# Maboroshi0327/MHAda-Style-Transfer

Measured on AMD Instinct MI355X. Metric: stylized frames/sec (whole job) at 512x512 batch 8 fp32 [configs[1]], higher is better.
Workload: dtype f32; 1 GPU; stylize 512x512 content+style, batch 8; resolution=512, batch_per_gpu=8, global_batch=8, compute_dtype=f32, parallelism=replicas x1

## Files before the change

### include/mhada_hip.h

```cpp
#ifndef MHADA_HIP_H
#define MHADA_HIP_H

#ifdef __cplusplus
extern "C" {
#endif

typedef void* mhada_stream_t;

enum { MHADA_OK = 0, MHADA_ERR_ARG = 1, MHADA_ERR_LAUNCH = 2 };
enum { MHADA_F32 = 0, MHADA_BF16 = 1 };
enum { MHADA_ACT_SOFTMAX = 0, MHADA_ACT_COSINE = 1 };
enum { MHADA_PAD_REFLECT = 0, MHADA_PAD_ZERO = 1 };
enum {
  MHADA_A_ROWS = 0,
  MHADA_A_PATCH8 = 1,
  MHADA_A_CONV3X3 = 2,
  MHADA_A_CONV3X3_UP2 = 3,
  MHADA_A_CONV3X3_ZERO = 4,
  MHADA_A_SPLIT3 = 5
};
enum { MHADA_BF16X3 = 2 };

int mhada_abi_version(void);
const char* mhada_last_error(void);
// ... 126 lines not shown
int mhada_colsum(const float* x, float* out, long long rows, int C, float* work, long long work_floats,
                 mhada_stream_t stream);

int mhada_layernorm_fwd(const float* x, float* y, float* stats, const float* gamma, const float* beta,
                        int rows, int cols, float eps, mhada_stream_t stream);
int mhada_layernorm_fwd_split3(const float* x, float* y, void* planes, float* stats, const float* gamma,
                               const float* beta, int rows, int cols, float eps, mhada_stream_t stream);

int mhada_layernorm_bwd(const float* x, const float* dy, const float* stats, const float* gamma, float* dx,
                        float* dgamma, float* dbeta, float* work, long long work_floats, int rows, int cols,
                        mhada_stream_t stream);

int mhada_instnorm_bwd(const float* dy, const float* y, const float* rstd, float* dx, double* work,
                       int B, int N, int C, int splits, mhada_stream_t stream);

int mhada_attn_train_bwd_prep(const float* dout, const float* x, const float* mo, float* dx, float* dmo,
                              float* dd, long long rows, mhada_stream_t stream);

int mhada_pos_embed_bwd(const float* g, float* gpos, int C, int bh, int bw, int oh, int ow,
                        mhada_stream_t stream);
long long mhada_feat_stats_work(int B, long long P, int C);
int mhada_feat_stats(const float* x, const float* t, float* mu, float* sd, float* mse, double* work,
                     long long work_doubles, int B, long long P, int C, mhada_stream_t stream);
int mhada_feat_loss_bwd(const float* x, const float* t, const float* mu, const float* alpha, const float* beta,
                        const float* kp, float ks, float* g, int B, long long P, int C, int relu, mhada_stream_t stream);
int mhada_relu_bwd(const float* dy, const float* y, float* dx, long long n, mhada_stream_t stream);
int mhada_reflect_fold(const float* dxp, float* dx, int B, int H, int W, int C, const float* relu_mask,
                       mhada_stream_t stream);
int mhada_maxpool2(const float* x, float* y, int B, int H, int W, int C, mhada_stream_t stream);
int mhada_maxpool2_bwd(const float* x, const float* dy, float* dx, int B, int H, int W, int C, int relu_mask,
                       mhada_stream_t stream);
int mhada_upsample2x_bwd(const float* dy, const float* relu_x, float* dx, int B, int H, int W, int C,
                         mhada_stream_t stream);
int mhada_vgg_input(const float* img, float* out, int B, int H, int W, int Cp, mhada_stream_t stream);
int mhada_vgg_input_bwd(const float* dout, float* dimg, int B, int H, int W, int Cp, mhada_stream_t stream);

int mhada_loss_attn(const float* q, const float* k, const float* v, const float* x, const float* x_mu,
                    const float* x_rs, float* out, int B, int Nq, int Ns, int Dqk, int Dv, int activation,
                    mhada_stream_t stream);
int mhada_rows_normalize(const float* x, const float* mu, const float* rs, float* out, int unit,
                         int B, int N, int C, mhada_stream_t stream);

int mhada_frame_ingest(const void* frames, int B, int H, int W, long long row_bytes, int bgr, float* out,
                       int Ho, int Wo, mhada_stream_t stream);

int mhada_wino_weights(const float* w, float* u, int Cout, int Cin, mhada_stream_t stream);
int mhada_conv3x3_wgrad_wino_splits(int B, int H, int W, int Cin, int Cout);
int mhada_conv3x3_wgrad_wino(const float* x, const float* g, float* dw, float* db, float* work, long long work_floats,
                             int B, int H, int W, int Cin, int Cout, long long ldg, int pad_mode,
                             mhada_stream_t stream);
int mhada_conv3x3_wino(const float* x, const float* u, const float* bias, float* y, int B, int H, int W,
                       int Cin, int Cout, long long ldc, int pad_mode, int pad, int relu,
                       const float* relu_mask, mhada_stream_t stream);

int mhada_vgg_stem_dgrad(const float* dy, const float* y, const float* wd, float* dimg, int B, int H, int W,
                         mhada_stream_t stream);
int mhada_out3_dgrad(const float* dy, const float* y, const float* wd, const float* relu_x, float* dx, int B, int H,
                     int W, mhada_stream_t stream);
long long mhada_out3_wgrad_work(int B, int H, int W);
int mhada_out3_wgrad(const float* x, const float* dy, const float* y, float* dw, float* db, float* work,
                     long long work_floats, int B, int H, int W, mhada_stream_t stream);

#ifdef __cplusplus
}
#endif
#endif
```

### mhada-style-transfer_amd/csrc/abi.hip

```cpp
#include "common.h"

#include <mutex>
#include <stdlib.h>
#include <string.h>

namespace mhada {

static thread_local std::string g_last_error;

void set_error(const std::string& msg) { g_last_error = msg; }

int fail(const std::string& msg) {
  set_error(msg);
  return MHADA_ERR_ARG;
}

int check_launch(const char* what) {
  const hipError_t e = hipGetLastError();
  if (e != hipSuccess) {
    set_error(std::string(what) + ": " + hipGetErrorString(e));
    return MHADA_ERR_LAUNCH;
  }
  return MHADA_OK;
}

namespace {
struct Knob {
  const char* name;
  int Tuning::*field;
};
const Knob kKnobs[] = {
    {"attn_fixed_shift", &Tuning::attn_fixed_shift}, {"attn_waves", &Tuning::attn_waves},
    {"attn_tk", &Tuning::attn_tk},                   {"attn_prio", &Tuning::attn_prio},
    {"vit_attn_vec", &Tuning::vit_attn_vec},         {"out3_mfma", &Tuning::out3_mfma},
    {"out3_tile", &Tuning::out3_tile},               {"gemm_pp", &Tuning::gemm_pp},
    {"gemm_persist", &Tuning::gemm_persist},         {"gemm_pp128", &Tuning::gemm_pp128},
    {"gemm_ldsepi", &Tuning::gemm_ldsepi},           {"gemm_n64", &Tuning::gemm_n64},
    {"conv_c64", &Tuning::conv_c64},                 {"conv_dir", &Tuning::conv_dir},                 {"gemm_rinit", &Tuning::gemm_rinit},
    {"tn_skinny_lds", &Tuning::tn_skinny_lds},       {"train_dkv_dma", &Tuning::train_dkv_dma},
    {"wino4", &Tuning::wino4},                       {"upsample_quad", &Tuning::upsample_quad},
    {"xknob", &Tuning::xknob},
};

Tuning g_tuning;
std::once_flag g_tuning_once;

void read_env_once() {
  std::call_once(g_tuning_once, [] {
    for (const Knob& k : kKnobs) {
      std::string env = "MHADA_";
      for (const char* c = k.name; *c; ++c) env += (char)(*c >= 'a' && *c <= 'z' ? *c - 32 : *c);
      if (const char* v = getenv(env.c_str())) g_tuning.*k.field = atoi(v);
    }
  });
}

bool valid(const char* name, int v) {
  if (!strcmp(name, "attn_waves")) return v == 0 || v == 4 || v == 8;
  if (!strcmp(name, "attn_tk")) return v == 64 || v == 128;
  if (!strcmp(name, "gemm_n64")) return v == 128 || v == 256;
  if (!strcmp(name, "xknob")) return v >= 0 && v < 16;
  return v == 0 || v == 1;
}
}

const Tuning& tuning() {
  read_env_once();
  return g_tuning;
}

}

extern "C" int mhada_abi_version(void) { return 16; }

extern "C" const char* mhada_last_error(void) { return mhada::g_last_error.c_str(); }

extern "C" int mhada_set_tuning(const char* name, int value) {
  using namespace mhada;
  read_env_once();
  if (!name) return fail("mhada_set_tuning: null name");
  for (const Knob& k : kKnobs) {
    if (!strcmp(k.name, name)) {
      if (!valid(name, value)) return fail(std::string("mhada_set_tuning: bad value for ") + name);
      g_tuning.*k.field = value;
      return MHADA_OK;
    }
  }
  return fail(std::string("mhada_set_tuning: unknown knob ") + name);
}

extern "C" int mhada_get_tuning(const char* name, int* value) {
  using namespace mhada;
  read_env_once();
  if (!name || !value) return fail("mhada_get_tuning: null argument");
  for (const Knob& k : kKnobs) {
    if (!strcmp(k.name, name)) {
      *value = g_tuning.*k.field;
      return MHADA_OK;
    }
  }
  return fail(std::string("mhada_get_tuning: unknown knob ") + name);
}
```

### mhada-style-transfer_amd/csrc/common.h

```cpp
#pragma once
#include <hip/hip_runtime.h>
#include <stdint.h>
#include <string>

#include "../../include/mhada_hip.h"

typedef __bf16 bf16;
typedef __bf16 bf16x8 __attribute__((ext_vector_type(8)));
typedef __bf16 bf16x4 __attribute__((ext_vector_type(4)));
typedef float f32x16 __attribute__((ext_vector_type(16)));
typedef float f32x4 __attribute__((ext_vector_type(4)));
typedef float f32x2 __attribute__((ext_vector_type(2)));

#define MHADA_DEV __device__ __forceinline__

namespace mhada {

void set_error(const std::string& msg);
int fail(const std::string& msg);
int check_launch(const char* what);

struct Tuning {
  int attn_fixed_shift = 1;
  int attn_waves = 0;
  int attn_tk = 128;
  int attn_prio = 1;
  int vit_attn_vec = 1;
  int out3_mfma = 1;
  int out3_tile = 1;
  int gemm_pp = 1;
  int gemm_persist = 1;
  int gemm_pp128 = 1;
  int gemm_ldsepi = 1;
  int gemm_n64 = 128;
  int conv_c64 = 1;
  int conv_dir = 1;
  int gemm_rinit = 1;
  int tn_skinny_lds = 1;
  int wino4 = 1;
  int train_dkv_dma = 1;
  int upsample_quad = 1;
  int xknob = 0;
};
const Tuning& tuning();

int conv3x3_c64(const void* x, const void* w, const float* bias, void* y, int B, int H, int W, bool up, int relu,
                hipStream_t s);
int conv3x3_dir(const void* x, const void* w, const float* bias, void* y, int B, int H, int W, int cin, int cout,
                int relu, hipStream_t s);

template <typename T> MHADA_DEV float to_f32(T x);
template <> MHADA_DEV float to_f32<float>(float x) { return x; }
template <> MHADA_DEV float to_f32<bf16>(bf16 x) { return (float)x; }

template <typename T> MHADA_DEV T from_f32(float x);
template <> MHADA_DEV float from_f32<float>(float x) { return x; }
template <> MHADA_DEV bf16 from_f32<bf16>(float x) { return (bf16)x; }

template <typename T> struct Vec16;
template <> struct Vec16<float> { typedef f32x4 type; static constexpr int N = 4; };
template <> struct Vec16<bf16> { typedef bf16x8 type; static constexpr int N = 8; };

MHADA_DEV float bilerp(float ly0, float ly1, float lx0, float lx1, float x00, float x01, float x10, float x11) {
  return fmaf(ly1, fmaf(lx0, x10, lx1 * x11), ly0 * fmaf(lx0, x00, lx1 * x01));
}

MHADA_DEV float wave_sum(float v) {
#pragma unroll
  for (int o = 32; o > 0; o >>= 1) v += __shfl_xor(v, o, 64);
  return v;
}
MHADA_DEV float wave_max(float v) {
#pragma unroll
  for (int o = 32; o > 0; o >>= 1) v = fmaxf(v, __shfl_xor(v, o, 64));
  return v;
}

MHADA_DEV int xcd_remap(int bid, int nblk) {
  const int q = nblk / 8, r = nblk % 8;
  const int xcd = bid % 8, k = bid / 8;
  return (xcd < r ? xcd * (q + 1) : r * (q + 1) + (xcd - r) * q) + k;
}

}
```

### mhada-style-transfer_amd/csrc/wino.hip

```cpp
#include "common.h"

#include <algorithm>
#include <utility>

#ifndef WINO_DBG
#define WINO_DBG 0
#endif
#ifndef WINO4_DBG
#define WINO4_DBG 0
#endif

namespace mhada {

namespace {
constexpr int kT = 8;
constexpr int kTT = kT * kT;
constexpr int kCO = 64;
constexpr int kCK = 8;
constexpr int kRP = 2 * kT + 2;
constexpr int kRaw = kRP * kRP;
constexpr int kRDma = (2 * kRaw + 63) / 64;
constexpr int kVS = 16 * kTT * kCK;
constexpr int kUS = 16 * kCO * kCK;
constexpr int kRS = kRDma * 64 * 4;
// ... 353 lines not shown
      if constexpr ((DBG & 4) == 0) {
#pragma unroll
        for (int s = 0; s < 4; ++s)
          acc[xi] = __builtin_amdgcn_mfma_f32_32x32x2f32(oa[xi % 3][s], ob[xi % 3][s], acc[xi], 0, 0, 0);
      }
      if (xi < 11) dma_piece(xi, k + 1, N, k + 2, C);
      if (xi == 2) tload(N);
      if (xi == 4) { tcols(); trows(N, 0); }
      if (xi == 5) trows(N, 2);
      fence();
    }
    publish();
  };
  int k = 0;
  for (; k + 1 < nck; k += 2) {
    chunk(k, std::integral_constant<int, 0>());
    chunk(k + 1, std::integral_constant<int, 1>());
  }
  if (k < nck) chunk(k, std::integral_constant<int, 0>());

  const int co = co0 + 32 * ch + r32;
  const float bias = p.bias ? p.bias[co] : 0.f;
#pragma unroll
  for (int r = 0; r < 16; ++r) {
    const int tile = 32 * th + (r & 3) + 8 * (r >> 2) + 4 * h;
    float m[4][2];
#pragma unroll
    for (int i = 0; i < 4; ++i) {
      const float m0 = acc[4 * i][r], m1 = acc[4 * i + 1][r], m2 = acc[4 * i + 2][r], m3 = acc[4 * i + 3][r];
      m[i][0] = m0 + m1 + m2;
      m[i][1] = m1 - m2 - m3;
    }
    const int oy0 = 2 * (by * kT + (tile >> 3)), ox0 = 2 * (bx * kT + (tile & 7));
#pragma unroll
    for (int q = 0; q < 2; ++q) {
      const float e1 = -m[2][q] - m[3][q];
      float y0 = m[0][q] + m[1][q] + m[2][q] + bias;
      float y1 = m[1][q] + e1 + bias;
      if (p.relu) {
        y0 = fmaxf(y0, 0.f);
        y1 = fmaxf(y1, 0.f);
      }
      const int ox = ox0 + q;
      if (ox < p.Wo) {
        const long long i0 = ((long long)(b * p.Ho + oy0) * p.Wo + ox) * p.ldc + co;
        const long long i1 = i0 + (long long)p.Wo * p.ldc;
        if (p.mask) {
          if (oy0 < p.Ho && !(p.mask[i0] > 0.f)) y0 = 0.f;
          if (oy0 + 1 < p.Ho && !(p.mask[i1] > 0.f)) y1 = 0.f;
        }
        if (oy0 < p.Ho) p.y[i0] = y0;
        if (oy0 + 1 < p.Ho) p.y[i1] = y1;
      }
    }
  }
}

__global__ void wino_weights_kernel(const float* __restrict__ w, float* __restrict__ u, int Cout, int Cin) {
  const long long i = (long long)blockIdx.x * blockDim.x + threadIdx.x;
  if (i >= (long long)Cout * Cin) return;
  const int ci = (int)(i % Cin), co = (int)(i / Cin);
  float g[9];
#pragma unroll
  for (int t = 0; t < 9; ++t) g[t] = w[((long long)co * 9 + t) * Cin + ci];
  float gg[12];
#pragma unroll
  for (int kx = 0; kx < 3; ++kx) {
    const float a = g[kx], bb = g[3 + kx], c = g[6 + kx];
    gg[0 * 3 + kx] = a;
    gg[1 * 3 + kx] = 0.5f * (a + bb + c);
    gg[2 * 3 + kx] = 0.5f * (a - bb + c);
    gg[3 * 3 + kx] = c;
  }
  float* ub = u + ((long long)(ci / kCK) * 16 * Cout + co) * kCK + (ci % kCK);
#pragma unroll
  for (int r = 0; r < 4; ++r) {
    const float a = gg[3 * r], bb = gg[3 * r + 1], c = gg[3 * r + 2];
    const float v[4] = {a, 0.5f * (a + bb + c), 0.5f * (a - bb + c), c};
#pragma unroll
    for (int j = 0; j < 4; ++j) ub[(long long)(4 * r + j) * Cout * kCK] = v[j];
  }
}
constexpr int kWgT = 8;
constexpr int kWgS = 16 * 64 * kWgT;
constexpr int kWgRX = 4 * 18 * 64;
constexpr int kWgRY = 2 * 16 * 64;

struct WgP {
  const float* x;
  const float* g;
  float* slab;
  float* cslab;
  int B, H, W, Cin, Cout, zero;
  long long ldg;
  int crow, nchunk, cps;
};

MHADA_DEV int wg_px(int px, int c) { return px * 64 + (c ^ (8 * ((px >> 1) & 7))); }

template <bool ZERO>
__global__ void __launch_bounds__(512, 1) wino_wgrad_kernel(const WgP p) {
  __shared__ __attribute__((aligned(16))) float lds[4 * kWgS + kWgRX + kWgRY];
  auto sYh = [&](int i) { return lds + i * kWgS; };
  auto sVb = [&](int i) { return lds + (2 + i) * kWgS; };
  float* sRX = lds + 4 * kWgS;
  float* sRY = sRX + kWgRX;
// ... 240 lines not shown
  if (B <= 0 || H < 2 || W < 16 || Cin <= 0 || Cout <= 0 || Cin % 64 || Cout % 64) return 0;
  const long long nchunk = (long long)B * (H / 2) * (W / 16);
  const long long blocks = (long long)(Cout / 64) * (Cin / 64);
  const long long s = std::max<long long>(1, std::min<long long>((512 + blocks - 1) / blocks, nchunk / 16));
  return (int)std::min<long long>(s, 65535);
}

extern "C" int mhada_conv3x3_wgrad_wino(const float* x, const float* g, float* dw, float* db, float* work,
                                        long long work_floats, int B, int H, int W, int Cin, int Cout, long long ldg,
                                        int pad_mode, mhada_stream_t s_) {
  if (!x || !g || !dw || !work || B <= 0 || H < 2 || W < 2 || Cin <= 0 || Cout <= 0)
    return fail("mhada_conv3x3_wgrad_wino: bad args");
  if (Cin % 64 || Cout % 64 || H % 2 || W % 16)
    return fail("mhada_conv3x3_wgrad_wino: needs Cin % 64 == 0, Cout % 64 == 0, H even, W % 16 == 0");
  if (pad_mode != MHADA_PAD_REFLECT && pad_mode != MHADA_PAD_ZERO) return fail("mhada_conv3x3_wgrad_wino: bad pad_mode");
  if (ldg < Cout || ldg % 4) return fail("mhada_conv3x3_wgrad_wino: ldg >= Cout, ldg % 4 == 0");
  if (((uintptr_t)x | (uintptr_t)g | (uintptr_t)work) & 15) return fail("mhada_conv3x3_wgrad_wino: 16-byte aligned x, g, work");
  if ((long long)B * H * W * std::max<long long>(Cin, ldg) > (1LL << 31) - 1)
    return fail("mhada_conv3x3_wgrad_wino: problem too large for 32-bit indexing");
  WgP p;
  p.x = x; p.g = g;
  p.B = B; p.H = H; p.W = W; p.Cin = Cin; p.Cout = Cout; p.ldg = ldg;
  p.zero = pad_mode == MHADA_PAD_ZERO;
  p.crow = W / 16;
  p.nchunk = B * (H / 2) * p.crow;
  int S = mhada_conv3x3_wgrad_wino_splits(B, H, W, Cin, Cout);
  const long long per = 16LL * Cout * Cin + (db ? Cout : 0);
  S = (int)std::min<long long>(S, work_floats / per);
  if (S < 1) return fail("mhada_conv3x3_wgrad_wino: workspace smaller than 16*Cout*Cin (+Cout) floats");
  p.cps = (p.nchunk + S - 1) / S;
  S = (p.nchunk + p.cps - 1) / p.cps;
  p.slab = work;
  p.cslab = db ? work + (long long)S * 16 * Cout * Cin : nullptr;
  const dim3 grid((unsigned)((Cout / 64) * (Cin / 64)), (unsigned)S);
  if (p.zero)
    hipLaunchKernelGGL(wino_wgrad_kernel<true>, grid, dim3(512), 0, (hipStream_t)s_, p);
  else
    hipLaunchKernelGGL(wino_wgrad_kernel<false>, grid, dim3(512), 0, (hipStream_t)s_, p);
  if (int rc = check_launch("mhada_conv3x3_wgrad_wino")) return rc;
  const long long n = (long long)Cout * Cin;
  hipLaunchKernelGGL(wino_wgrad_finish_kernel, dim3((unsigned)((n + 255) / 256)), dim3(256), 0, (hipStream_t)s_,
                     p.slab, p.cslab, dw, db, Cout, Cin, S);
  return check_launch("mhada_conv3x3_wgrad_wino(finish)");
}

extern "C" int mhada_wino_weights(const float* w, float* u, int Cout, int Cin, mhada_stream_t s_) {
  if (!w || !u || Cout <= 0 || Cin <= 0 || Cin % kCK) return fail("mhada_wino_weights: bad args (Cin % 8 == 0)");
  const long long n = (long long)Cout * Cin;
  hipLaunchKernelGGL(wino_weights_kernel, dim3((unsigned)((n + 255) / 256)), dim3(256), 0, (hipStream_t)s_, w, u,
                     Cout, Cin);
  return check_launch("mhada_wino_weights");
}

extern "C" int mhada_conv3x3_wino(const float* x, const float* u, const float* bias, float* y, int B, int H, int W,
                                  int Cin, int Cout, long long ldc, int pad_mode, int pad, int relu,
                                  const float* relu_mask, mhada_stream_t s_) {
  if (!x || !u || !y || B <= 0 || H < 2 || W < 2 || Cin <= 0 || Cout <= 0)
    return fail("mhada_conv3x3_wino: bad args");
  if (Cin % kCK || Cout % kCO) return fail("mhada_conv3x3_wino: needs Cin % 8 == 0 and Cout % 64 == 0");
  if (pad_mode != MHADA_PAD_REFLECT && pad_mode != MHADA_PAD_ZERO) return fail("mhada_conv3x3_wino: bad pad_mode");
  if (pad_mode == MHADA_PAD_ZERO && pad != 1 && pad != 2) return fail("mhada_conv3x3_wino: zero pad must be 1 or 2");
  if (ldc < Cout) return fail("mhada_conv3x3_wino: ldc < Cout");
  if (((uintptr_t)x | (uintptr_t)u) & 15) return fail("mhada_conv3x3_wino: x and u must be 16-byte aligned");
  WinoP p;
  p.x = x; p.u = u; p.bias = bias; p.y = y; p.mask = relu_mask;
  p.B = B; p.H = H; p.W = W; p.Cin = Cin; p.Cout = Cout;
  p.zero = pad_mode == MHADA_PAD_ZERO;
  p.pad = p.zero ? pad : 1;
  p.Ho = p.zero ? H + 2 * (pad - 1) : H;
  p.Wo = p.zero ? W + 2 * (pad - 1) : W;
  p.relu = relu;
  p.ldc = ldc;
  const int TY = (p.Ho + 1) / 2, TX = (p.Wo + 1) / 2;
  p.nby = (TY + kT - 1) / kT;
  p.nbx = (TX + kT - 1) / kT;
  p.nbn = Cout / kCO;
  const long long nblk = (long long)B * p.nby * p.nbx * p.nbn;
  if (nblk > (1LL << 31) - 1 || (long long)B * H * W * Cin > (1LL << 31) - 1)
    return fail("mhada_conv3x3_wino: problem too large for 32-bit indexing");
  p.nblk = (int)nblk;
  if (tuning().wino4 && (long long)B * H * W * Cin * 4 < 0x7ff00000LL) {
    hipLaunchKernelGGL(wino4_kernel<WINO4_DBG>, dim3(p.nblk), dim3(256), 0, (hipStream_t)s_, p);
  } else
    hipLaunchKernelGGL(wino_kernel, dim3(p.nblk), dim3(512), 0, (hipStream_t)s_, p);
  return check_launch("mhada_conv3x3_wino");
}
```

### mhada-style-transfer_amd/mhada_hip/_lib.py

```python
from __future__ import annotations

import ctypes
import os
import threading

LIB_PATH = os.path.join(os.path.dirname(os.path.abspath(__file__)), "libmhada_hip.so")

F32, BF16 = 0, 1
ACT_SOFTMAX, ACT_COSINE = 0, 1
A_ROWS, A_PATCH8, A_CONV3X3, A_CONV3X3_UP2, A_CONV3X3_ZERO, A_SPLIT3 = 0, 1, 2, 3, 4, 5
BF16X3 = 2
PAD_REFLECT, PAD_ZERO = 0, 1

_c_ll = ctypes.c_longlong
_vp = ctypes.c_void_p


class GemmArgs(ctypes.Structure):
    _fields_ = [
        ("M", ctypes.c_int), ("N", ctypes.c_int), ("K", ctypes.c_int),
        ("nb1", ctypes.c_int), ("nb2", ctypes.c_int),
        ("compute", ctypes.c_int), ("a_mode", ctypes.c_int),
        ("a", _vp), ("a_dtype", ctypes.c_int), ("lda", _c_ll), ("sa1", _c_ll), ("sa2", _c_ll),
        ("a_mu", _vp), ("smu1", _c_ll), ("smu2", _c_ll),
# ... 34 lines not shown
    "mhada_fold_block": (_I, [_vp] * 12 + [_F, _I, _I, _I, _vp]),
    "mhada_transpose_v": (_I, [_vp, _vp, _I, _I, _I, _I, _vp]),
    "mhada_cosine_prep": (_I, [_vp, _vp, _I, _I, _I, _I, _I, _vp]),
    "mhada_cosine_moments": (_I, [_vp, _vp, _I, _I, _I, _I, _vp, _vp, _I, _vp]),
    "mhada_cosine_attn": (_I, [_vp, _vp, _vp, _vp, _vp, _vp, _vp, _I, _I, _I, _I, _vp]),
    "mhada_attn": (_I, [_vp] * 8 + [_I, _I, _I, _I, _I, _I, _vp]),
    "mhada_split3_kv": (_I, [_vp, _vp, _vp, _I, _I, _I, _vp]),
    "mhada_kv_proj_split3": (_I, [_vp] * 5 + [_I, _I, _I, _vp]),
    "mhada_split3_rows": (_I, [_vp, _vp, _c_ll, _vp]),
    "mhada_split3_weight": (_I, [_vp, _vp, _I, _I, _I, _vp]),
    "mhada_attn_split3": (_I, [_vp] * 7 + [_I, _I, _I, _I, _vp]),
    "mhada_attn_train_fwd": (_I, [_vp] * 7 + [_I, _I, _I, _vp]),
    "mhada_attn_train_fwd_vt": (_I, [_vp] * 8 + [_I, _I, _I, _vp]),
    "mhada_attn_train_fwd_split3": (_I, [_vp] * 8 + [_I, _I, _I, _vp]),
    "mhada_transpose64": (_I, [_vp, _vp, _I, _I, _I, _vp]),
    "mhada_gemm_n64_split3": (_I, [_vp, _vp, _vp, _I, _I, _I, _I, _c_ll, _I, _c_ll, _c_ll, _I, _c_ll, _vp]),
    "mhada_transpose64_split3": (_I, [_vp, _vp, _I, _I, _I, _vp]),
    "mhada_attn_train_bwd": (_I, [_vp] * 9 + [_I, _I, _I, _vp]),
    "mhada_attn_train_dkv": (_I, [_vp] * 9 + [_I, _I, _I, _vp]),
    "mhada_conv3x3_out3": (_I, [_vp, _I, _vp, _vp, _vp, _I, _I, _I, _I, _I, _vp]),
    "mhada_upsample2x": (_I, [_vp, _vp, _I, _I, _I, _I, _I, _vp]),
    "mhada_warp": (_I, [_vp, _vp, _vp, _I, _I, _I, _I, _I, _vp]),
    "mhada_warp_bwd": (_I, [_vp, _vp, _vp, _I, _I, _I, _I, _I, _vp]),
    "mhada_flow_warp_mask": (_I, [_vp, _vp, _vp, _I, _I, _F, _I, _vp]),
    "mhada_warp_l1": (_I, [_vp, _vp, _vp, _vp, _vp, _vp, _I, _I, _I, _I, _vp]),
    "mhada_frame_ingest": (_I, [_vp, _I, _I, _I, _c_ll, _I, _vp, _I, _I, _vp]),
    "mhada_gemm_tn_splits": (_I, [_I, _I, _I]),
    "mhada_loss_attn": (_I, [_vp] * 7 + [_I, _I, _I, _I, _I, _I, _vp]),
    "mhada_rows_normalize": (_I, [_vp] * 4 + [_I, _I, _I, _I, _vp]),
    "mhada_gemm_tn": (_I, [ctypes.POINTER(GemmTnArgs), _vp, _c_ll, _vp]),
    "mhada_colsum": (_I, [_vp, _vp, _c_ll, _I, _vp, _c_ll, _vp]),
    "mhada_layernorm_fwd": (_I, [_vp, _vp, _vp, _vp, _vp, _I, _I, _F, _vp]),
    "mhada_layernorm_fwd_split3": (_I, [_vp, _vp, _vp, _vp, _vp, _vp, _I, _I, _F, _vp]),
    "mhada_layernorm_bwd": (_I, [_vp, _vp, _vp, _vp, _vp, _vp, _vp, _vp, _c_ll, _I, _I, _vp]),
    "mhada_pos_embed_bwd": (_I, [_vp, _vp, _I, _I, _I, _I, _I, _vp]),
    "mhada_instnorm_bwd": (_I, [_vp, _vp, _vp, _vp, _vp, _I, _I, _I, _I, _vp]),
    "mhada_attn_train_bwd_prep": (_I, [_vp, _vp, _vp, _vp, _vp, _vp, _c_ll, _vp]),
    "mhada_vit_batch_attn_bwd": (_I, [_vp, _vp, _vp, _I, _I, _I, _I, _vp]),
    "mhada_vit_batch_attn_bwd_split3": (_I, [_vp, _vp, _vp, _vp, _c_ll, _I, _I, _I, _I, _vp]),
    "mhada_relu_bwd": (_I, [_vp, _vp, _vp, _c_ll, _vp]),
    "mhada_feat_stats_work": (_c_ll, [_I, _c_ll, _I]),
    "mhada_feat_stats": (_I, [_vp, _vp, _vp, _vp, _vp, _vp, _c_ll, _I, _c_ll, _I, _vp]),
    "mhada_feat_loss_bwd": (_I, [_vp, _vp, _vp, _vp, _vp, _vp, _F, _vp, _I, _c_ll, _I, _I, _vp]),
    "mhada_reflect_fold": (_I, [_vp, _vp, _I, _I, _I, _I, _vp, _vp]),
    "mhada_maxpool2": (_I, [_vp, _vp, _I, _I, _I, _I, _vp]),
    "mhada_maxpool2_bwd": (_I, [_vp, _vp, _vp, _I, _I, _I, _I, _I, _vp]),
    "mhada_upsample2x_bwd": (_I, [_vp, _vp, _vp, _I, _I, _I, _I, _vp]),
    "mhada_vgg_input": (_I, [_vp, _vp, _I, _I, _I, _I, _vp]),
    "mhada_vgg_input_bwd": (_I, [_vp, _vp, _I, _I, _I, _I, _vp]),
    "mhada_wino_weights": (_I, [_vp, _vp, _I, _I, _vp]),
    "mhada_conv3x3_wgrad_wino_splits": (_I, [_I, _I, _I, _I, _I]),
    "mhada_conv3x3_wgrad_wino": (_I, [_vp, _vp, _vp, _vp, _vp, _c_ll, _I, _I, _I, _I, _I, _c_ll, _I, _vp]),
    "mhada_conv3x3_wino": (_I, [_vp] * 4 + [_I] * 5 + [_c_ll, _I, _I, _I, _vp, _vp]),
    "mhada_vgg_stem_dgrad": (_I, [_vp] * 4 + [_I] * 3 + [_vp]),
    "mhada_out3_dgrad": (_I, [_vp] * 5 + [_I] * 3 + [_vp]),
    "mhada_out3_wgrad_work": (_c_ll, [_I, _I, _I]),
    "mhada_out3_wgrad": (_I, [_vp] * 6 + [_c_ll, _I, _I, _I, _vp]),
}

_lib = None
_lock = threading.Lock()


def load(path: str | None = None) -> ctypes.CDLL:
    global _lib
    if _lib is not None and path is None:
        return _lib
    with _lock:
        if _lib is not None and path is None:
            return _lib
        p = path or LIB_PATH
        if not os.path.exists(p):
            raise RuntimeError(
                f"MHAda HIP library not found at {p}; build it with "
                "`python -c 'import __graft_entry__ as g; g.build()'` (make -C mhada-style-transfer_amd/csrc)")
        lib = ctypes.CDLL(p)
        for name, (res, args) in SIGNATURES.items():
            fn = getattr(lib, name)
            fn.restype = res
            fn.argtypes = args
        if path is None:
            _lib = lib
        return lib


ABI_VERSION = 16


def get_tuning(name: str) -> int:
    v = ctypes.c_int()
    check(load().mhada_get_tuning(name.encode(), ctypes.byref(v)), "mhada_get_tuning")
    return v.value


def set_tuning(name: str, value: int) -> None:
    check(load().mhada_set_tuning(name.encode(), int(value)), "mhada_set_tuning")


class tuning:

    def __init__(self, **knobs: int):
        self.knobs = knobs
        self.saved = {}

    def __enter__(self):
        for k, v in self.knobs.items():
            self.saved[k] = get_tuning(k)
            set_tuning(k, v)
        return self

    def __exit__(self, *exc):
        for k, v in self.saved.items():
            set_tuning(k, v)
        return False


def check(rc: int, what: str) -> None:
    if rc != 0:
        msg = load().mhada_last_error()
        msg = msg.decode() if msg else "unknown error"
        if rc == 1:
            raise ValueError(f"{what}: {msg}")
        raise RuntimeError(f"{what}: {msg}")
```

### mhada-style-transfer_amd/mhada_hip/ops.py

```python
from __future__ import annotations

import contextlib
import ctypes
from typing import Optional

import torch

from . import _lib
from ._lib import A_CONV3X3, A_CONV3X3_UP2, A_CONV3X3_ZERO, A_PATCH8, A_ROWS, A_SPLIT3, BF16, BF16X3, F32, GemmArgs, GemmTnArgs

_DT = {torch.float32: F32, torch.bfloat16: BF16}


def dt_code(dtype: torch.dtype) -> int:
    try:
        return _DT[dtype]
    except KeyError:
        raise ValueError(f"unsupported dtype {dtype}; the HIP path computes in float32 or bfloat16")


def _ptr(t: Optional[torch.Tensor]) -> Optional[int]:
    return None if t is None else t.data_ptr()


# ... 91 lines not shown


def patch_embed(img: torch.Tensor, w: torch.Tensor, bias: torch.Tensor, pos: Optional[torch.Tensor],
                patch: int = 8) -> torch.Tensor:
    if patch != 8:
        raise ValueError("the HIP patch embedding implements patch_size=8 (the reference default)")
    B, Ci, H, W = img.shape
    h, wd = H // 8, W // 8
    N, C = h * wd, w.shape[0]
    out = torch.empty(B, N, C, device=img.device, dtype=torch.float32)
    return gemm(a=img, w=w, c=out, M=N, N=C, K=Ci * 64, compute=w.dtype, a_mode=A_PATCH8,
                sa=(Ci * H * W, 0), nb=(B, 1), img=(Ci, H, W), ldw=w.stride(0), bias=bias,
                r=pos, ldr=C, sr=(0, 0), ldc=C, sc=(N * C, 0))


WINO = True


def wino_eligible(x: torch.Tensor, w: torch.Tensor, upsample: bool) -> bool:
    return (WINO and w.dtype == torch.float32 and x.dtype == torch.float32 and not upsample
            and x.shape[-1] % 8 == 0 and w.shape[0] % 64 == 0 and x.shape[1] >= 2 and x.shape[2] >= 2
            and x.numel() < 2 ** 31 and x.numel() // x.shape[-1] * w.shape[0] < 2 ** 31)


WINO_WGRAD = True


def wgrad_wino_eligible(x: torch.Tensor, g: torch.Tensor, cout: int) -> bool:
    if not (WINO_WGRAD and x.is_cuda and x.dtype == torch.float32 and g.dtype == torch.float32):
        return False
    B, H, W, ci = x.shape
    return (ci % 64 == 0 and cout % 64 == 0 and H % 2 == 0 and W % 16 == 0 and g.shape[:3] == x.shape[:3]
            and g.shape[3] >= cout and g.shape[3] % 4 == 0 and x.is_contiguous() and g.is_contiguous()
            and B * H * W * max(ci, g.shape[3]) < 2 ** 31)


def conv3x3_wgrad_wino(x: torch.Tensor, g: torch.Tensor, cout: int, pad_mode: str = "reflect",
                       bias: bool = True):
    _need_gpu(x, g)
    B, H, W, ci = x.shape
    lib = _lib.load()
    S = lib.mhada_conv3x3_wgrad_wino_splits(B, H, W, ci, cout)
    if S <= 0:
        raise ValueError("conv3x3_wgrad_wino: ineligible shape")
    work = torch.empty(S * (16 * cout * ci + (cout if bias else 0)), device=x.device, dtype=torch.float32)
    dw = torch.empty(cout, 9 * ci, device=x.device, dtype=torch.float32)
    db = torch.empty(cout, device=x.device, dtype=torch.float32) if bias else None
    _call("mhada_conv3x3_wgrad_wino", x, x.data_ptr(), g.data_ptr(), dw.data_ptr(),
          db.data_ptr() if bias else None, work.data_ptr(), work.numel(), B, H, W, ci, cout, g.shape[3],
          _lib.PAD_REFLECT if pad_mode == "reflect" else _lib.PAD_ZERO)
    return dw, db


def wino_weights(w: torch.Tensor) -> torch.Tensor:
    _need_gpu(w)
    Co, K = w.shape
    Ci = K // 9
    if w.dtype != torch.float32 or K != 9 * Ci or not w.is_contiguous():
        raise ValueError("wino_weights needs a contiguous fp32 [Cout][9*Cin] weight")
    u = torch.empty(Ci // 8, 16, Co, 8, device=w.device, dtype=torch.float32)
    _call("mhada_wino_weights", w, w.data_ptr(), u.data_ptr(), Co, Ci)
    return u


def conv3x3_wino(x: torch.Tensor, u: torch.Tensor, bias: Optional[torch.Tensor], relu: bool = True,
                 pad_mode: str = "reflect", pad: int = 1, out: Optional[torch.Tensor] = None,
                 relu_mask: Optional[torch.Tensor] = None) -> torch.Tensor:
    _need_gpu(x, u, bias, out, relu_mask)
    B, H, W, Ci = x.shape
    Co = u.shape[2]
    if x.dtype != torch.float32 or not x.is_contiguous() or u.shape[0] * 8 != Ci:
        raise ValueError("conv3x3_wino: contiguous fp32 NHWC input matching the filters")
    if pad_mode == "reflect":
        mode, Ho, Wo, pad = _lib.PAD_REFLECT, H, W, 1
    elif pad_mode == "zero":
        mode, Ho, Wo = _lib.PAD_ZERO, H + 2 * (pad - 1), W + 2 * (pad - 1)
    else:
        raise ValueError(f"pad_mode {pad_mode!r}")
    y = torch.empty(B, Ho, Wo, Co, device=x.device, dtype=torch.float32) if out is None else out
    if y.shape[:3] != (B, Ho, Wo) or y.dtype != torch.float32 or y.shape[-1] < Co or not y.is_contiguous():
        raise ValueError("conv3x3_wino: bad output buffer")
    if relu_mask is not None and (relu_mask.shape != y.shape or relu_mask.dtype != torch.float32
                                  or not relu_mask.is_contiguous()):
        raise ValueError("conv3x3_wino: relu_mask must be a contiguous fp32 tensor shaped like the output")
    _call("mhada_conv3x3_wino", x, x.data_ptr(), u.data_ptr(), _ptr(bias), y.data_ptr(), B, H, W, Ci, Co,
          y.shape[-1], mode, pad, int(relu), _ptr(relu_mask))
    return y


def conv3x3(x: torch.Tensor, w: torch.Tensor, bias: Optional[torch.Tensor], out_dtype: torch.dtype,
            upsample: bool, relu: bool = True, pad_mode: str = "reflect", pad: int = 1,
            out: Optional[torch.Tensor] = None, wino_u: Optional[torch.Tensor] = None,
            relu_mask: Optional[torch.Tensor] = None) -> torch.Tensor:
    B, H, W, Ci = x.shape
    Co = w.shape[0]
    if out_dtype == torch.float32 and wino_eligible(x, w, upsample) and x.is_contiguous():
        u = wino_u if wino_u is not None else wino_weights(w)
        return conv3x3_wino(x, u, bias, relu, pad_mode, pad, out, relu_mask)
    if relu_mask is not None:
        return relu_bwd(conv3x3(x, w, bias, out_dtype, upsample, relu, pad_mode, pad, out), relu_mask)
    if pad_mode == "zero":
        if upsample:
            raise ValueError("zero-padded conv3x3 has no fused upsample")
        Ho, Wo = H + 2 * (pad - 1), W + 2 * (pad - 1)
        mode = A_CONV3X3_ZERO
    elif pad_mode == "reflect":
        Ho, Wo = (2 * H, 2 * W) if upsample else (H, W)
        mode = A_CONV3X3_UP2 if upsample else A_CONV3X3
        pad = 0
    else:
        raise ValueError(f"pad_mode {pad_mode!r}")
    y = torch.empty(B, Ho, Wo, Co, device=x.device, dtype=out_dtype) if out is None else out
    return gemm(a=x, w=w, c=y, M=B * Ho * Wo, N=Co, K=9 * Ci, compute=w.dtype, a_mode=mode, img=(Ci, H, W),
                ldw=w.stride(0), bias=bias, ldc=y.shape[-1], relu=relu, pad=pad)


def upsample2x(x: torch.Tensor) -> torch.Tensor:
    _need_gpu(x)
    B, H, W, C = x.shape
    y = torch.empty(B, 2 * H, 2 * W, C, device=x.device, dtype=x.dtype)
    _call("mhada_upsample2x", x, x.data_ptr(), y.data_ptr(), dt_code(x.dtype), B, H, W, C)
    return y


def conv3x3_out3(x: torch.Tensor, w: torch.Tensor, bias: torch.Tensor, clamp255: bool = False) -> torch.Tensor:
    B, H, W, Ci = x.shape
    _need_gpu(x, w, bias)
    y = torch.empty(B, 3, H, W, device=x.device, dtype=torch.float32)
    _call("mhada_conv3x3_out3", x, x.data_ptr(), dt_code(x.dtype), w.data_ptr(), bias.data_ptr(),
                                        y.data_ptr(), B, H, W, Ci, int(clamp255))
    return y


def layernorm(x: torch.Tensor, g: torch.Tensor, b: torch.Tensor, out_dtype: torch.dtype, eps: float) -> torch.Tensor:
    _need_gpu(x, g, b)
    rows, cols = x.shape
    y = torch.empty(rows, cols, device=x.device, dtype=out_dtype)
    _call("mhada_layernorm", x, x.data_ptr(), y.data_ptr(), dt_code(out_dtype), g.data_ptr(), b.data_ptr(),
                                     rows, cols, eps)
# ... 749 lines not shown
```

Baseline: 321.4 frames/s.

## Add split-bf16x3 MFMA Winograd conv3x3 kernel with pre-split transformed weights

```diff
diff --git a/include/mhada_hip.h b/include/mhada_hip.h
--- a/include/mhada_hip.h
+++ b/include/mhada_hip.h
@@ -202,6 +202,10 @@
 int mhada_conv3x3_wino(const float* x, const float* u, const float* bias, float* y, int B, int H, int W,
                        int Cin, int Cout, long long ldc, int pad_mode, int pad, int relu,
                        const float* relu_mask, mhada_stream_t stream);
+int mhada_wino_weights_split3(const float* w, void* up, int Cout, int Cin, mhada_stream_t stream);
+int mhada_conv3x3_wino_split3(const float* x, const float* u, const void* up, const float* bias, float* y, int B,
+                              int H, int W, int Cin, int Cout, long long ldc, int pad_mode, int pad, int relu,
+                              const float* relu_mask, mhada_stream_t stream);
 
 int mhada_vgg_stem_dgrad(const float* dy, const float* y, const float* wd, float* dimg, int B, int H, int W,
                          mhada_stream_t stream);
diff --git a/mhada-style-transfer_amd/csrc/abi.hip b/mhada-style-transfer_amd/csrc/abi.hip
--- a/mhada-style-transfer_amd/csrc/abi.hip
+++ b/mhada-style-transfer_amd/csrc/abi.hip
@@ -38,6 +38,7 @@
     {"gemm_ldsepi", &Tuning::gemm_ldsepi},           {"gemm_n64", &Tuning::gemm_n64},
     {"conv_c64", &Tuning::conv_c64},                 {"conv_dir", &Tuning::conv_dir},                 {"gemm_rinit", &Tuning::gemm_rinit},
     {"tn_skinny_lds", &Tuning::tn_skinny_lds},       {"train_dkv_dma", &Tuning::train_dkv_dma},
+    {"wino_split3", &Tuning::wino_split3},
     {"wino4", &Tuning::wino4},                       {"upsample_quad", &Tuning::upsample_quad},
     {"xknob", &Tuning::xknob},
 };
@@ -71,7 +72,7 @@
 
 }
 
-extern "C" int mhada_abi_version(void) { return 16; }
+extern "C" int mhada_abi_version(void) { return 17; }
 
 extern "C" const char* mhada_last_error(void) { return mhada::g_last_error.c_str(); }
 
diff --git a/mhada-style-transfer_amd/csrc/common.h b/mhada-style-transfer_amd/csrc/common.h
--- a/mhada-style-transfer_amd/csrc/common.h
+++ b/mhada-style-transfer_amd/csrc/common.h
@@ -38,6 +38,7 @@
   int gemm_rinit = 1;
   int tn_skinny_lds = 1;
   int wino4 = 1;
+  int wino_split3 = 1;
   int train_dkv_dma = 1;
   int upsample_quad = 1;
   int xknob = 0;
diff --git a/mhada-style-transfer_amd/csrc/wino.hip b/mhada-style-transfer_amd/csrc/wino.hip
--- a/mhada-style-transfer_amd/csrc/wino.hip
+++ b/mhada-style-transfer_amd/csrc/wino.hip
@@ -429,6 +429,256 @@
         if (oy0 < p.Ho) p.y[i0] = y0;
         if (oy0 + 1 < p.Ho) p.y[i1] = y1;
       }
+    }
+  }
+}
+
+constexpr int kSK = 16;
+constexpr int kSImg = 64 * kSK * 2;
+constexpr int kSStage = 12 * kSImg;
+constexpr int kSRDma = (4 * kRaw + 63) / 64;
+constexpr int kSRawB = kSRDma * 1024;
+
+struct WinoS3P : WinoP {
+  const bf16* up;
+};
+
+MHADA_DEV int rpix(int pix) { return pix ^ ((pix >> 2) & 1); }
+
+__global__ void __launch_bounds__(256, 1) wino_s3_kernel(const WinoS3P p) {
+  __shared__ __attribute__((aligned(16))) unsigned char sV0[kSStage];
+  __shared__ __attribute__((aligned(16))) unsigned char sV1[kSStage];
+  __shared__ __attribute__((aligned(16))) unsigned char sU0[kSStage];
+  __shared__ __attribute__((aligned(16))) unsigned char sU1[kSStage];
+  __shared__ __attribute__((aligned(16))) unsigned char sR0[kSRawB];
+  __shared__ __attribute__((aligned(16))) unsigned char sR1[kSRawB];
+  const int tid = threadIdx.x, lane = tid & 63, h = lane >> 5, r32 = lane & 31;
+  const int wave = __builtin_amdgcn_readfirstlane(tid >> 6);
+  const int th = wave & 1, ch = wave >> 1;
+
+  int id = xcd_remap(blockIdx.x, p.nblk);
+  const int nsp = p.nblk / p.nbn;
+  const int nb = id / nsp;
+  id -= nb * nsp;
+  const int bx = id % p.nbx;
+  id /= p.nbx;
+  const int by = id % p.nby;
+  const int b = id / p.nby;
+  const int co0 = nb * kCO;
+  const int P = p.zero ? p.pad : 1;
+  const int nck = p.Cin / kSK, nst = 4 * nck;
+
+  const __amdgpu_buffer_rsrc_t xr = __builtin_amdgcn_make_buffer_rsrc(
+      const_cast<float*>(p.x), 0, (int)((long long)p.B * p.H * p.W * p.Cin * 4), 0x00020000);
+  const __amdgpu_buffer_rsrc_t ur =
+      __builtin_amdgcn_make_buffer_rsrc(const_cast<bf16*>(p.up), 0, p.Cin * p.Cout * 96, 0x00020000);
+  int rvo[6];
+#pragma unroll
+  for (int t = 0; t < 6; ++t) {
+    const int slot = 64 * (wave + 4 * t) + lane;
+    const int pix = rpix(slot >> 2);
+    int iy = 2 * by * kT - P + pix / kRP, ix = 2 * bx * kT - P + pix % kRP;
+    bool inside = pix < kRaw;
+    if (p.zero) {
+      inside = inside && iy >= 0 && iy < p.H && ix >= 0 && ix < p.W;
+    } else {
+      iy = reflect_clamp(iy, p.H);
+      ix = reflect_clamp(ix, p.W);
+    }
+    rvo[t] = inside ? (((b * p.H + iy) * p.W + ix) * p.Cin + 4 * (slot & 3)) * 4 : 0x7ff00000;
+  }
+  int uvo[6];
+#pragma unroll
+  for (int t = 0; t < 6; ++t) {
+    const int slot = 64 * (6 * wave + t) + lane;
+    const int g = slot >> 7, row = (slot >> 1) & 63, sh = slot & 1;
+    uvo[t] = ((g * p.Cout + co0 + row) * kSK + 8 * (sh ^ ((row >> 3) & 1))) * 2;
+  }
+  const int usb = 12 * p.Cout * kSK * 2;
+  typedef __attribute__((address_space(3))) void* LdsP;
+
+  const int tq = tid & 3, tt = tid >> 2;
+  int roffs[16];
+#pragma unroll
+  for (int i = 0; i < 4; ++i)
+#pragma unroll
+    for (int j = 0; j < 4; ++j) roffs[4 * i + j] = rpix((2 * (tt >> 3) + i) * kRP + 2 * (tt & 7) + j) * 64 + tq * 16;
+  const int vdst = tt * 32 + ((((tq >> 1) ^ (tt >> 3)) & 1) << 4) + (tq & 1) * 8;
+  auto transform = [&](auto ic, const unsigned char* sr, unsigned char* sv) {
+    constexpr int I = decltype(ic)::value;
+    constexpr int RA = I == 0 ? 0 : (I == 2 ? 2 : 1), RB = I == 0 ? 2 : (I == 1 ? 2 : (I == 2 ? 1 : 3));
+    f32x4 t[4];
+#pragma unroll
+    for (int j = 0; j < 4; ++j) {
+      const f32x4 a = *reinterpret_cast<const f32x4*>(sr + roffs[4 * RA + j]);
+      const f32x4 c = *reinterpret_cast<const f32x4*>(sr + roffs[4 * RB + j]);
+      t[j] = I == 1 ? a + c : a - c;
+    }
+    const f32x4 v[4] = {t[0] - t[2], t[1] + t[2], t[2] - t[1], t[1] - t[3]};
+#pragma unroll
+    for (int x = 0; x < 4; ++x) {
+      bf16x4 p0, p1, p2;
+#pragma unroll
+      for (int e = 0; e < 4; ++e) {
+        const bf16 a = (bf16)v[x][e];
+        const float r = v[x][e] - (float)a;
+        const bf16 c = (bf16)r;
+        p0[e] = a;
+        p1[e] = c;
+        p2[e] = (bf16)(r - (float)c);
+      }
+      *reinterpret_cast<bf16x4*>(sv + (3 * x + 0) * kSImg + vdst) = p0;
+      *reinterpret_cast<bf16x4*>(sv + (3 * x + 1) * kSImg + vdst) = p1;
+      *reinterpret_cast<bf16x4*>(sv + (3 * x + 2) * kSImg + vdst) = p2;
+    }
+  };
+
+  f32x16 acc[16];
+#pragma unroll
+  for (int x = 0; x < 16; ++x)
+#pragma unroll
+    for (int q = 0; q < 16; ++q) acc[x][q] = 0.f;
+  const int fsw = (h ^ ((r32 >> 3) & 1)) << 4;
+  const int aoff = (32 * th + r32) * 32 + fsw, boff = (32 * ch + r32) * 32 + fsw;
+  auto mfmas = [&](auto ic, const unsigned char* sv, const unsigned char* su) {
+    constexpr int I = decltype(ic)::value;
+    constexpr int TA[6] = {1, 2, 0, 1, 0, 0}, TB[6] = {1, 0, 2, 0, 1, 0};
+#pragma unroll
+    for (int pr = 0; pr < 2; ++pr) {
+      bf16x8 a[2][3], bq[2][3];
+#pragma unroll
+      for (int x = 0; x < 2; ++x)
+#pragma unroll
+        for (int pl = 0; pl < 3; ++pl) {
+          a[x][pl] = *reinterpret_cast<const bf16x8*>(sv + (3 * (2 * pr + x) + pl) * kSImg + aoff);
+          bq[x][pl] = *reinterpret_cast<const bf16x8*>(su + (3 * (2 * pr + x) + pl) * kSImg + boff);
+        }
+#pragma unroll
+      for (int t = 0; t < 6; ++t)
+#pragma unroll
+        for (int x = 0; x < 2; ++x)
+          acc[4 * I + 2 * pr + x] =
+              __builtin_amdgcn_mfma_f32_32x32x16_bf16(a[x][TA[t]], bq[x][TB[t]], acc[4 * I + 2 * pr + x], 0, 0, 0);
+    }
+  };
+  auto publish = [&]() {
+    __builtin_amdgcn_sched_barrier(0);
+    asm volatile("s_waitcnt vmcnt(0)" ::: "memory");
+    __syncthreads();
+  };
+  auto dma_u = [&](int s, unsigned char* su) {
+    const int so = min(s, nst - 1) * usb;
+#pragma unroll
+    for (int t = 0; t < 6; ++t)
+      __builtin_amdgcn_raw_ptr_buffer_load_lds(ur, (LdsP)(su + (6 * wave + t) * 1024), 16, (unsigned)uvo[t], so, 0, 0);
+  };
+  auto dma_raw = [&](int t0, int k, unsigned char* sr) {
+    const int so = min(k, nck - 1) * kSK * 4;
+#pragma unroll
+    for (int t = t0; t < t0 + 3; ++t)
+      if (t < 5 || wave == 0)
+        __builtin_amdgcn_raw_ptr_buffer_load_lds(xr, (LdsP)(sr + (wave + 4 * t) * 1024), 16, (unsigned)rvo[t], so, 0, 0);
+  };
+
+  dma_u(0, sU0);
+  dma_raw(0, 0, sR0);
+  dma_raw(3, 0, sR0);
+  publish();
+  transform(std::integral_constant<int, 0>(), sR0, sV0);
+  __syncthreads();
+  auto stage = [&](int k, auto ic, auto cc) {
+    constexpr int I = decltype(ic)::value, C = decltype(cc)::value;
+    unsigned char* const svn = (I & 1) ? sV0 : sV1;
+    dma_u(4 * k + I + 1, (I & 1) ? sU0 : sU1);
+    if constexpr (I < 2) dma_raw(3 * I, k + 1, C ? sR0 : sR1);
+    __builtin_amdgcn_sched_barrier(0);
+    if constexpr (I < 3)
+      transform(std::integral_constant<int, I + 1>(), C ? sR1 : sR0, svn);
+    else
+      transform(std::integral_constant<int, 0>(), C ? sR0 : sR1, svn);
+    mfmas(ic, (I & 1) ? sV1 : sV0, (I & 1) ? sU1 : sU0);
+    publish();
+  };
+  auto chunk = [&](int k, auto cc) {
+    stage(k, std::integral_constant<int, 0>(), cc);
+    stage(k, std::integral_constant<int, 1>(), cc);
+    stage(k, std::integral_constant<int, 2>(), cc);
+    stage(k, std::integral_constant<int, 3>(), cc);
+  };
+  int k = 0;
+  for (; k + 1 < nck; k += 2) {
+    chunk(k, std::integral_constant<int, 0>());
+    chunk(k + 1, std::integral_constant<int, 1>());
+  }
+  if (k < nck) chunk(k, std::integral_constant<int, 0>());
+
+  const int co = co0 + 32 * ch + r32;
+  const float bias = p.bias ? p.bias[co] : 0.f;
+#pragma unroll
+  for (int r = 0; r < 16; ++r) {
+    const int tile = 32 * th + (r & 3) + 8 * (r >> 2) + 4 * h;
+    float m[4][2];
+#pragma unroll
+    for (int i = 0; i < 4; ++i) {
+      const float m0 = acc[4 * i][r], m1 = acc[4 * i + 1][r], m2 = acc[4 * i + 2][r], m3 = acc[4 * i + 3][r];
+      m[i][0] = m0 + m1 + m2;
+      m[i][1] = m1 - m2 - m3;
+    }
+    const int oy0 = 2 * (by * kT + (tile >> 3)), ox0 = 2 * (bx * kT + (tile & 7));
+#pragma unroll
+    for (int q = 0; q < 2; ++q) {
+      const float e1 = -m[2][q] - m[3][q];
+      float y0 = m[0][q] + m[1][q] + m[2][q] + bias;
+      float y1 = m[1][q] + e1 + bias;
+      if (p.relu) {
+        y0 = fmaxf(y0, 0.f);
+        y1 = fmaxf(y1, 0.f);
+      }
+      const int ox = ox0 + q;
+      if (ox < p.Wo) {
+        const long long i0 = ((long long)(b * p.Ho + oy0) * p.Wo + ox) * p.ldc + co;
+        const long long i1 = i0 + (long long)p.Wo * p.ldc;
+        if (p.mask) {
+          if (oy0 < p.Ho && !(p.mask[i0] > 0.f)) y0 = 0.f;
+          if (oy0 + 1 < p.Ho && !(p.mask[i1] > 0.f)) y1 = 0.f;
+        }
+        if (oy0 < p.Ho) p.y[i0] = y0;
+        if (oy0 + 1 < p.Ho) p.y[i1] = y1;
+      }
+    }
+  }
+}
+
+__global__ void wino_weights_s3_kernel(const float* __restrict__ w, bf16* __restrict__ up, int Cout, int Cin) {
+  const long long i = (long long)blockIdx.x * blockDim.x + threadIdx.x;
+  if (i >= (long long)Cout * Cin) return;
+  const int ci = (int)(i % Cin), co = (int)(i / Cin);
+  float g[9];
+#pragma unroll
+  for (int t = 0; t < 9; ++t) g[t] = w[((long long)co * 9 + t) * Cin + ci];
+  float gg[12];
+#pragma unroll
+  for (int kx = 0; kx < 3; ++kx) {
+    const float a = g[kx], bb = g[3 + kx], c = g[6 + kx];
+    gg[0 * 3 + kx] = a;
+    gg[1 * 3 + kx] = 0.5f * (a + bb + c);
+    gg[2 * 3 + kx] = 0.5f * (a - bb + c);
+    gg[3 * 3 + kx] = c;
+  }
+  bf16* ub = up + ((long long)(ci / kSK) * 48 * Cout + co) * kSK + (ci % kSK);
+#pragma unroll
+  for (int r = 0; r < 4; ++r) {
+    const float a = gg[3 * r], bb = gg[3 * r + 1], c = gg[3 * r + 2];
+    const float v[4] = {a, 0.5f * (a + bb + c), 0.5f * (a - bb + c), c};
+#pragma unroll
+    for (int j = 0; j < 4; ++j) {
+      const bf16 p0 = (bf16)v[j];
+      const float r1 = v[j] - (float)p0;
+      const bf16 p1 = (bf16)r1;
+      bf16* o = ub + (long long)(4 * r + j) * 3 * Cout * kSK;
+      o[0] = p0;
+      o[(long long)Cout * kSK] = p1;
+      o[2LL * Cout * kSK] = (bf16)(r1 - (float)p1);
     }
   }
 }
@@ -775,9 +1025,9 @@
   return check_launch("mhada_wino_weights");
 }
 
-extern "C" int mhada_conv3x3_wino(const float* x, const float* u, const float* bias, float* y, int B, int H, int W,
-                                  int Cin, int Cout, long long ldc, int pad_mode, int pad, int relu,
-                                  const float* relu_mask, mhada_stream_t s_) {
+static int conv3x3_wino_launch(const float* x, const float* u, const void* up, const float* bias, float* y, int B,
+                               int H, int W, int Cin, int Cout, long long ldc, int pad_mode, int pad, int relu,
+                               const float* relu_mask, mhada_stream_t s_) {
   if (!x || !u || !y || B <= 0 || H < 2 || W < 2 || Cin <= 0 || Cout <= 0)
     return fail("mhada_conv3x3_wino: bad args");
   if (Cin % kCK || Cout % kCO) return fail("mhada_conv3x3_wino: needs Cin % 8 == 0 and Cout % 64 == 0");
@@ -802,9 +1052,37 @@
   if (nblk > (1LL << 31) - 1 || (long long)B * H * W * Cin > (1LL << 31) - 1)
     return fail("mhada_conv3x3_wino: problem too large for 32-bit indexing");
   p.nblk = (int)nblk;
-  if (tuning().wino4 && (long long)B * H * W * Cin * 4 < 0x7ff00000LL) {
+  const bool bufx = (long long)B * H * W * Cin * 4 < 0x7ff00000LL;
+  if (up && tuning().wino_split3 && Cin % kSK == 0 && bufx && (long long)Cin * Cout * 96 < 0x7ff00000LL) {
+    if ((uintptr_t)up & 15) return fail("mhada_conv3x3_wino_split3: up must be 16-byte aligned");
+    WinoS3P q;
+    static_cast<WinoP&>(q) = p;
+    q.up = (const bf16*)up;
+    hipLaunchKernelGGL(wino_s3_kernel, dim3(p.nblk), dim3(256), 0, (hipStream_t)s_, q);
+  } else if (tuning().wino4 && bufx) {
     hipLaunchKernelGGL(wino4_kernel<WINO4_DBG>, dim3(p.nblk), dim3(256), 0, (hipStream_t)s_, p);
   } else
     hipLaunchKernelGGL(wino_kernel, dim3(p.nblk), dim3(512), 0, (hipStream_t)s_, p);
   return check_launch("mhada_conv3x3_wino");
 }
+
+extern "C" int mhada_conv3x3_wino(const float* x, const float* u, const float* bias, float* y, int B, int H, int W,
+                                  int Cin, int Cout, long long ldc, int pad_mode, int pad, int relu,
+                                  const float* relu_mask, mhada_stream_t s_) {
+  return conv3x3_wino_launch(x, u, nullptr, bias, y, B, H, W, Cin, Cout, ldc, pad_mode, pad, relu, relu_mask, s_);
+}
+
+extern "C" int mhada_conv3x3_wino_split3(const float* x, const float* u, const void* up, const float* bias, float* y,
+                                         int B, int H, int W, int Cin, int Cout, long long ldc, int pad_mode, int pad,
+                                         int relu, const float* relu_mask, mhada_stream_t s_) {
+  if (!up) return fail("mhada_conv3x3_wino_split3: bad args");
+  return conv3x3_wino_launch(x, u, up, bias, y, B, H, W, Cin, Cout, ldc, pad_mode, pad, relu, relu_mask, s_);
+}
+
+extern "C" int mhada_wino_weights_split3(const float* w, void* up, int Cout, int Cin, mhada_stream_t s_) {
+  if (!w || !up || Cout <= 0 || Cin <= 0 || Cin % kSK) return fail("mhada_wino_weights_split3: bad args (Cin % 16 == 0)");
+  const long long n = (long long)Cout * Cin;
+  hipLaunchKernelGGL(wino_weights_s3_kernel, dim3((unsigned)((n + 255) / 256)), dim3(256), 0, (hipStream_t)s_, w,
+                     (bf16*)up, Cout, Cin);
+  return check_launch("mhada_wino_weights_split3");
+}
diff --git a/mhada-style-transfer_amd/mhada_hip/_lib.py b/mhada-style-transfer_amd/mhada_hip/_lib.py
--- a/mhada-style-transfer_amd/mhada_hip/_lib.py
+++ b/mhada-style-transfer_amd/mhada_hip/_lib.py
@@ -110,6 +110,8 @@
     "mhada_conv3x3_wgrad_wino_splits": (_I, [_I, _I, _I, _I, _I]),
     "mhada_conv3x3_wgrad_wino": (_I, [_vp, _vp, _vp, _vp, _vp, _c_ll, _I, _I, _I, _I, _I, _c_ll, _I, _vp]),
     "mhada_conv3x3_wino": (_I, [_vp] * 4 + [_I] * 5 + [_c_ll, _I, _I, _I, _vp, _vp]),
+    "mhada_conv3x3_wino_split3": (_I, [_vp] * 5 + [_I] * 5 + [_c_ll, _I, _I, _I, _vp, _vp]),
+    "mhada_wino_weights_split3": (_I, [_vp, _vp, _I, _I, _vp]),
     "mhada_vgg_stem_dgrad": (_I, [_vp] * 4 + [_I] * 3 + [_vp]),
     "mhada_out3_dgrad": (_I, [_vp] * 5 + [_I] * 3 + [_vp]),
     "mhada_out3_wgrad_work": (_c_ll, [_I, _I, _I]),
@@ -142,7 +144,7 @@
         return lib
 
 
-ABI_VERSION = 16
+ABI_VERSION = 17
 
 
 def get_tuning(name: str) -> int:
diff --git a/mhada-style-transfer_amd/mhada_hip/ops.py b/mhada-style-transfer_amd/mhada_hip/ops.py
--- a/mhada-style-transfer_amd/mhada_hip/ops.py
+++ b/mhada-style-transfer_amd/mhada_hip/ops.py
@@ -167,6 +167,17 @@
     return dw, db
 
 
+def wino_weights_split3(w: torch.Tensor) -> torch.Tensor:
+    _need_gpu(w)
+    Co, K = w.shape
+    Ci = K // 9
+    if w.dtype != torch.float32 or K != 9 * Ci or Ci % 16 or not w.is_contiguous():
+        raise ValueError("wino_weights_split3 needs a contiguous fp32 [Cout][9*Cin] weight, Cin % 16 == 0")
+    up = torch.empty(Ci // 16, 16, 3, Co, 16, device=w.device, dtype=torch.bfloat16)
+    _call("mhada_wino_weights_split3", w, w.data_ptr(), up.data_ptr(), Co, Ci)
+    return up
+
+
 def wino_weights(w: torch.Tensor) -> torch.Tensor:
     _need_gpu(w)
     Co, K = w.shape
@@ -175,6 +186,8 @@
         raise ValueError("wino_weights needs a contiguous fp32 [Cout][9*Cin] weight")
     u = torch.empty(Ci // 8, 16, Co, 8, device=w.device, dtype=torch.float32)
     _call("mhada_wino_weights", w, w.data_ptr(), u.data_ptr(), Co, Ci)
+    if Ci % 16 == 0:
+        u.split3 = wino_weights_split3(w)
     return u
 
 
@@ -198,8 +211,13 @@
     if relu_mask is not None and (relu_mask.shape != y.shape or relu_mask.dtype != torch.float32
                                   or not relu_mask.is_contiguous()):
         raise ValueError("conv3x3_wino: relu_mask must be a contiguous fp32 tensor shaped like the output")
-    _call("mhada_conv3x3_wino", x, x.data_ptr(), u.data_ptr(), _ptr(bias), y.data_ptr(), B, H, W, Ci, Co,
-          y.shape[-1], mode, pad, int(relu), _ptr(relu_mask))
+    up = getattr(u, "split3", None)
+    if up is not None:
+        _call("mhada_conv3x3_wino_split3", x, x.data_ptr(), u.data_ptr(), up.data_ptr(), _ptr(bias), y.data_ptr(),
+              B, H, W, Ci, Co, y.shape[-1], mode, pad, int(relu), _ptr(relu_mask))
+    else:
+        _call("mhada_conv3x3_wino", x, x.data_ptr(), u.data_ptr(), _ptr(bias), y.data_ptr(), B, H, W, Ci, Co,
+              y.shape[-1], mode, pad, int(relu), _ptr(relu_mask))
     return y
 
 
```

Result: faster. 328.8 frames/s, median of 6 (+2.3%).
